# xhuan8/SoccerPlayerShapePose

Hardware: NVIDIA B200
Metric: SMPL meshes/sec fwd+bwd (higher is better)
Workload: dtype f32 (bf16x3 split on tcgen05, fp32 accumulate)

## Files before the change

soccerplayershapepose_b200/csrc/blend_umma.cu:

```cuda
#include <cuda.h>
#include <algorithm>

#include "umma_common.cuh"

namespace b200smpl {

template <int BN>
__global__ void __launch_bounds__(GEMM_THREADS, 1)
umma_gemm2_kernel(const __grid_constant__ GemmOps ops, int split3, int ntiles, int nc8, int slab_begin, int slab_end,
                  int slabs_per_split, float* __restrict__ D, int ldd, long long split_stride) {
  constexpr int BNH = BN / 2;
  constexpr int A_BYTES = BM * BK * 2, B_BYTES = BNH * BK * 2;
  static_assert(B_BYTES % 1024 == 0, "the 128-byte swizzle needs every stage offset 1024-byte aligned");
  constexpr int MAX_STAGES = 6;
  constexpr uint32_t TMEM_COLS = 256;
  const int stage_bytes = (split3 ? 2 : 1) * (A_BYTES + B_BYTES);
  const int nstages = split3 ? 3 : 6;
  extern __shared__ unsigned char smem_dyn[];
  unsigned char* smem = reinterpret_cast<unsigned char*>((reinterpret_cast<uintptr_t>(smem_dyn) + 1023) & ~(uintptr_t)1023);
  uint64_t* full_bar = reinterpret_cast<uint64_t*>(smem + MAX_STAGES * (A_BYTES + B_BYTES));
  uint64_t* peer_full_bar = full_bar + MAX_STAGES;
  uint64_t* empty_bar = peer_full_bar + MAX_STAGES;
  uint64_t* tmem_full_bar = empty_bar + MAX_STAGES;
  uint32_t* tmem_slot = reinterpret_cast<uint32_t*>(tmem_full_bar + 1);
// ... 104 lines not shown
      for (int c0 = 0; c0 < BN; c0 += 32) {
        uint32_t v[32];
        tmem_ld_32x32(tmem_base + ((uint32_t)(q * 32) << 16) + (uint32_t)c0, v);
        float* o = drow + c0;
#pragma unroll
        for (int i = 0; i < 32; i += 4)
          if (c0 + i < BN)
            *reinterpret_cast<uint4*>(o + i) = make_uint4(v[i], v[i + 1], v[i + 2], v[i + 3]);
      }
    } else {
#pragma unroll 1
      for (int c0 = 0; c0 < BN; c0 += 4) *reinterpret_cast<uint4*>(drow + c0) = make_uint4(0u, 0u, 0u, 0u);
    }
  }
  tc_fence_before();
  cluster_sync_all();
  if (warp == 1) {
    tc_fence_after();
    asm volatile("tcgen05.dealloc.cta_group::2.sync.aligned.b32 %0, %1;" ::"r"(tmem_base), "r"(TMEM_COLS) : "memory");
  }
}

constexpr int WS_STAGES = 5;
constexpr int WS_MAX_SLABS = 9;
constexpr int WS_BN = 128;


template <int DUMMY>
__global__ void __launch_bounds__(GEMM_THREADS, 1)
blend_fwd_bs2_kernel(const __grid_constant__ CUtensorMap map_w, const __grid_constant__ CUtensorMap map_f, int pslabs,
                     int ksteps_cs, int ksteps_p, int use_lo, int row0, int mtiles, int ntiles_n,
                     const __grid_constant__ BsWork work, float4* __restrict__ vpB, int nc4) {
  constexpr int SLAB = BM * BK * 2;
  constexpr int KS = BK / UMMA_K;
  constexpr uint32_t TMEM_COLS = 512;
  const int nslab_f = 1 + 2 * pslabs;
  const int nslab_w = 1 + (use_lo ? 2 : 1) * pslabs;
  extern __shared__ unsigned char smem_dyn[];
  unsigned char* smem = reinterpret_cast<unsigned char*>((reinterpret_cast<uintptr_t>(smem_dyn) + 1023) & ~(uintptr_t)1023);
  unsigned char* f_s = smem;
  unsigned char* w_s = smem + WS_MAX_SLABS * SLAB;
  uint64_t* bars = reinterpret_cast<uint64_t*>(w_s + WS_STAGES * SLAB);
  uint64_t* f_full = bars;
  uint64_t* peer_f_full = bars + 1;
  uint64_t* full_bar = bars + 2;
  uint64_t* peer_full_bar = full_bar + WS_STAGES;
  uint64_t* empty_bar = peer_full_bar + WS_STAGES;
  uint64_t* tfull_bar = empty_bar + WS_STAGES;
  uint64_t* tempty_bar = tfull_bar + 2;
  uint32_t* tmem_slot = reinterpret_cast<uint32_t*>(tempty_bar + 2);

  const int warp = threadIdx.x >> 5, lane = threadIdx.x & 31;
  const uint32_t rank = cluster_ctarank();
  const int piece = (int)(blockIdx.x >> 1);
  const int btile = (int)work.bp[piece] * 2 + (int)rank;
  const int wtp_begin = work.w0[piece], wtp_end = work.w1[piece];

  if (warp == 0 && lane == 0) {
    prefetch_tmap(&map_w);
    prefetch_tmap(&map_f);
  }
  if (warp == 1 && lane == 0) {
    mbar_init(f_full, 1);
    mbar_init(peer_f_full, 1);
    for (int i = 0; i < WS_STAGES; ++i) {
      mbar_init(&full_bar[i], 1);
      mbar_init(&peer_full_bar[i], 1);
      mbar_init(&empty_bar[i], 1);
    }
    for (int i = 0; i < 2; ++i) {
      mbar_init(&tfull_bar[i], 1);
      mbar_init(&tempty_bar[i], 8);
    }
    fence_barrier_init();
  }
  if (warp == 1) {
    __syncwarp();
    asm volatile("tcgen05.alloc.cta_group::2.sync.aligned.shared::cta.b32 [%0], %1;" ::"r"(smem_u32(tmem_slot)), "r"(TMEM_COLS)
                 : "memory");
    asm volatile("tcgen05.relinquish_alloc_permit.cta_group::2.sync.aligned;" ::: "memory");
  }
  tc_fence_before();
  cluster_sync_all();
  tc_fence_after();
  const uint32_t tmem_base = *tmem_slot;
  pdl_wait();
  if (threadIdx.x == 0) pdl_trigger();

  if (warp == 0) {
    if (elect_one()) {
      mbar_arrive_expect_tx(f_full, (uint32_t)nslab_f * SLAB);
      for (int s = 0; s < nslab_f; ++s) tma_load_2d(f_s + s * SLAB, &map_f, f_full, s * BK, btile * WS_BN);
    }
    __syncwarp();
    const uint64_t pol_keep = l2_policy_evict_last();
    int stage = 0;
    uint32_t phase = 0;
    for (int wtp = wtp_begin; wtp < wtp_end; ++wtp)
      for (int s = 0; s < nslab_w; ++s) {
        mbar_wait(&empty_bar[stage], phase ^ 1);
        if (elect_one()) {
          mbar_arrive_expect_tx(&full_bar[stage], SLAB);
          tma_load_2d_hint(w_s + stage * SLAB, &map_w, &full_bar[stage], s * BK, row0 + (wtp * 2 + (int)rank) * BM, pol_keep);
        }
        __syncwarp();
        if (++stage == WS_STAGES) { stage = 0; phase ^= 1; }
      }
  } else if (warp == 1) {
    int stage = 0;
    uint32_t phase = 0;
    if (rank == 0) {
      constexpr uint32_t idesc = make_idesc(2 * BM, 2 * WS_BN);
      mbar_wait(f_full, 0);
      mbar_wait(peer_f_full, 0);
      uint32_t tph0 = 0, tph1 = 0;
      int acc = 0;
      for (int wtp = wtp_begin; wtp < wtp_end; ++wtp, acc ^= 1) {
        const uint32_t tph = acc ? tph1 : tph0;
        mbar_wait(&tempty_bar[acc], tph ^ 1);
        if (acc) tph1 ^= 1; else tph0 ^= 1;
        tc_fence_after();
        const uint32_t d_tmem = tmem_base + (uint32_t)(acc * 2 * WS_BN);
        for (int s = 0; s < nslab_w; ++s) {
          mbar_wait(&full_bar[stage], phase);
          mbar_wait(&peer_full_bar[stage], phase);
          tc_fence_after();
          const uint64_t db = make_sw128_desc(smem_u32(w_s + stage * SLAB));
          int ks = ksteps_cs, f0 = 0, f1 = -1;
          if (s > 0) {
            const int j = (s - 1) % pslabs;
            ks = min(KS, ksteps_p - j * KS);
            f0 = 1 + j;
            if (s <= pslabs) f1 = 1 + pslabs + j;
          }
          const uint64_t da0 = make_sw128_desc(smem_u32(f_s + f0 * SLAB));
          const uint64_t da1 = make_sw128_desc(smem_u32(f_s + max(f1, 0) * SLAB));
          if (elect_one()) {
#pragma unroll
            for (int k = 0; k < KS; ++k)
              if (k < ks) umma_bf16_2cta(d_tmem, da0 + 2 * k, db + 2 * k, idesc, (s | k) != 0);
            if (f1 >= 0) {
#pragma unroll
              for (int k = 0; k < KS; ++k)
                if (k < ks) umma_bf16_2cta(d_tmem, da1 + 2 * k, db + 2 * k, idesc, 1u);
            }
            umma_commit_2cta(&empty_bar[stage]);
            if (s == nslab_w - 1) umma_commit_2cta(&tfull_bar[acc]);
          }
          __syncwarp();
          if (++stage == WS_STAGES) { stage = 0; phase ^= 1; }
        }
      }
    } else {
      mbar_wait(f_full, 0);
      if (elect_one()) remote_arrive(peer_f_full, 0);
      __syncwarp();
      for (int wtp = wtp_begin; wtp < wtp_end; ++wtp)
        for (int s = 0; s < nslab_w; ++s) {
          mbar_wait(&full_bar[stage], phase);
          if (elect_one()) remote_arrive(&peer_full_bar[stage], 0);
          __syncwarp();
          if (++stage == WS_STAGES) { stage = 0; phase ^= 1; }
        }
    }
  } else {
    const int q = warp & 3;
    uint32_t tph0 = 0, tph1 = 0;
    int acc = 0;
    for (int wtp = wtp_begin; wtp < wtp_end; ++wtp, acc ^= 1) {
      const uint32_t tph = acc ? tph1 : tph0;
      mbar_wait(&tfull_bar[acc], tph);
      if (acc) tph1 ^= 1; else tph0 ^= 1;
      tc_fence_after();
      if (btile < ntiles_n) {
        const bool live_hi = wtp * 2 + 1 < mtiles;
        float4* colbase = vpB + ((size_t)(btile * 4 + q) * nc4 + ((row0 + wtp * 2 * BM) >> 2)) * 32 + lane;
#pragma unroll 1
        for (int c0 = 0; c0 < 2 * WS_BN; c0 += 32) {
          if (c0 >= WS_BN && !live_hi) continue;
          uint32_t v[32];
          tmem_ld_32x32(tmem_base + ((uint32_t)(q * 32) << 16) + (uint32_t)(acc * 2 * WS_BN + c0), v);
// ... 16 lines not shown
  cluster_sync_all();
  if (warp == 1) {
    tc_fence_after();
    asm volatile("tcgen05.dealloc.cta_group::2.sync.aligned.b32 %0, %1;" ::"r"(tmem_base), "r"(TMEM_COLS) : "memory");
  }
}

typedef CUresult (*EncodeTiledFn)(CUtensorMap*, CUtensorMapDataType, cuuint32_t, void*, const cuuint64_t*,
                                  const cuuint64_t*, const cuuint32_t*, const cuuint32_t*, CUtensorMapInterleave,
                                  CUtensorMapSwizzle, CUtensorMapL2promotion, CUtensorMapFloatOOBfill);

static EncodeTiledFn get_encode_fn() {
  static EncodeTiledFn fn = nullptr;
  if (fn == nullptr) {
    void* p = nullptr;
    cudaDriverEntryPointQueryResult qres;
    if (cudaGetDriverEntryPoint("cuTensorMapEncodeTiled", &p, cudaEnableDefault, &qres) == cudaSuccess &&
        qres == cudaDriverEntryPointSuccess)
      fn = reinterpret_cast<EncodeTiledFn>(p);
  }
  return fn;
}

int make_map(CUtensorMap* map, const void* base, int k_extent, int rows, int pitch_elems, int box_rows) {
  EncodeTiledFn fn = get_encode_fn();
  if (fn == nullptr) return fail(B200SMPL_ERR_CUDA, "cuTensorMapEncodeTiled entry point not available");
  cuuint64_t dims[2] = {(cuuint64_t)k_extent, (cuuint64_t)rows};
  cuuint64_t strides[1] = {(cuuint64_t)pitch_elems * 2};
  cuuint32_t box[2] = {(cuuint32_t)BK, (cuuint32_t)box_rows};
  cuuint32_t estr[2] = {1, 1};
  CUresult r = fn(map, CU_TENSOR_MAP_DATA_TYPE_BFLOAT16, 2, const_cast<void*>(base), dims, strides, box, estr,
                  CU_TENSOR_MAP_INTERLEAVE_NONE, CU_TENSOR_MAP_SWIZZLE_128B, CU_TENSOR_MAP_L2_PROMOTION_L2_256B,
                  CU_TENSOR_MAP_FLOAT_OOB_FILL_NONE);
  if (r != CUDA_SUCCESS) return fail(B200SMPL_ERR_CUDA, "cuTensorMapEncodeTiled failed with code " + std::to_string((int)r));
  return 0;
}

int build_bs_work(int bp_total, int wtp_total, int tpcs, BsWork& work) {
  if (bp_total < 1 || wtp_total < 1) return -1;
  const long long total = (long long)bp_total * wtp_total;
  const int nranges = (int)std::min<long long>(total, std::max(tpcs, bp_total));
  struct Piece { int bp, w0, w1; };
  std::vector<Piece> pieces;
  for (int r = 0; r < nranges; ++r) {
    long long lo = total * r / nranges, hi = total * (r + 1) / nranges;
    while (lo < hi) {
      const int bp = (int)(lo / wtp_total);
      const long long end = std::min<long long>(hi, (long long)(bp + 1) * wtp_total);
      pieces.push_back({bp, (int)(lo - (long long)bp * wtp_total), (int)(end - (long long)bp * wtp_total)});
      lo = end;
    }
  }
  const int rect_chunks = std::max(1, std::min(wtp_total, tpcs / std::max(1, bp_total)));
  const int rect_len = (wtp_total + rect_chunks - 1) / rect_chunks;
  const int flat_len = (int)((total + nranges - 1) / nranges);
  if ((int)pieces.size() > BS_MAX_WORK || rect_len <= flat_len + 1) {
    pieces.clear();
    const int chunks = std::max(1, std::min(rect_chunks, BS_MAX_WORK / bp_total));
    const int wpc = (wtp_total + chunks - 1) / chunks;
    for (int bp = 0; bp < bp_total; ++bp)
      for (int w = 0; w < wtp_total; w += wpc) pieces.push_back({bp, w, std::min(wtp_total, w + wpc)});
    if ((int)pieces.size() > BS_MAX_WORK) return -1;
  }
  std::stable_sort(pieces.begin(), pieces.end(), [](const Piece& a, const Piece& b) { return a.w1 - a.w0 > b.w1 - b.w0; });
  memset(&work, 0, sizeof(work));
  int npieces = 0;
  for (const Piece& pc : pieces) {
    work.bp[npieces] = (uint16_t)pc.bp; work.w0[npieces] = (uint16_t)pc.w0; work.w1[npieces] = (uint16_t)pc.w1;
    ++npieces;
  }
  return npieces;
}

int launch_blend_fwd_umma(const DevModel& m, int mode, const __nv_bfloat16* feat, int S, int Sw, float* vpT,
                          int row_begin, int row_end, int num_sms, cudaStream_t st) {
  const int pslabs = m.fl.pseg / BK;
  const int use_lo = (mode == B200SMPL_MODE_BF16) ? 0 : 1;
  if (1 + 2 * pslabs > WS_MAX_SLABS) return fail(B200SMPL_ERR_INVALID, "feature pitch too large for the resident operand");
  CUtensorMap map_w, map_f;
  int rc;
  if ((rc = make_map(&map_w, m.Wf, m.fl.pitch, m.n_pad, m.fl.pitch, BM))) return rc;
  if ((rc = make_map(&map_f, feat, m.fl.pitch, Sw, m.fl.pitch, WS_BN))) return rc;
  constexpr int smem = (WS_MAX_SLABS + WS_STAGES) * BM * BK * 2 + 1024 + 256;
  auto kern = blend_fwd_bs2_kernel<0>;
  B200_SMEM_ATTR_ONCE(kern, smem);
  const int mtiles = (row_end - row_begin) / BM;
  const int wtp_total = (mtiles + 1) / 2;
  const int ntiles_n = Sw / WS_BN;
  const int bp_total = (ntiles_n + 1) / 2;
  BsWork work;
  const int npieces = build_bs_work(bp_total, wtp_total, std::max(1, num_sms / 2), work);
  if (npieces < 0) return fail(B200SMPL_ERR_INVALID, "slab too wide for the forward GEMM work list");
  cudaLaunchConfig_t cfg;
  memset(&cfg, 0, sizeof(cfg));
  cfg.gridDim = dim3(2 * npieces, 1, 1);
  cfg.blockDim = dim3(GEMM_THREADS, 1, 1);
  cfg.dynamicSmemBytes = smem;
  cfg.stream = st;
  cudaLaunchAttribute attr[2];
  attr[0].id = cudaLaunchAttributeClusterDimension;
  attr[0].val.clusterDim.x = 2;
  attr[0].val.clusterDim.y = 1;
  attr[0].val.clusterDim.z = 1;
  attr[1].id = cudaLaunchAttributeProgrammaticStreamSerialization;
  attr[1].val.programmaticStreamSerializationAllowed = 1;
  cfg.attrs = attr;
  cfg.numAttrs = pdl_enabled() ? 2 : 1;
  LaunchTimer _timer("blend_fwd_umma", st);
  B200_CUDA_TRY(cudaLaunchKernelEx(&cfg, kern, map_w, map_f, pslabs, (m.fl.k_cs + UMMA_K - 1) / UMMA_K,
                                   (NPOSE + UMMA_K - 1) / UMMA_K, use_lo, row_begin, mtiles, ntiles_n, work,
                                   reinterpret_cast<float4*>(vpT), m.n_pad / 4));
  B200_LAUNCH_CHECK("blend_fwd_umma");
  return 0;
}

}
extern "C" int b200smpl_debug_fwd_gemm_worklist(int body_tiles, int row_tiles, int num_sms, uint16_t* out, int capacity) {
  using namespace b200smpl;
  BsWork work;
  const int n = build_bs_work((body_tiles + 1) / 2, (row_tiles + 1) / 2, std::max(1, num_sms / 2), work);
  if (n < 0 || out == nullptr || n > capacity) return n < 0 ? -1 : n;
  for (int c = 0; c < n; ++c) { out[c * 3] = work.bp[c]; out[c * 3 + 1] = work.w0[c]; out[c * 3 + 2] = work.w1[c]; }
  return n;
}
namespace b200smpl {

int blend_bwd_umma_splits(const DevModel& m, int S, int num_sms) {
  const int mtiles = round_up((S + BM - 1) / BM, 2);
  const int slabs = (m.n_rows + BK - 1) / BK;
  int want = std::max(1, num_sms / mtiles);
  want = std::max(1, std::min(want, slabs / 8));
  return want;
}

// ... 52 lines not shown
```

soccerplayershapepose_b200/csrc/fused_fwd.cu:

```cuda
#include <algorithm>

#include "lbs_tiles.cuh"
#include "umma_common.cuh"

namespace b200smpl {

constexpr int FF_BN = 96;
constexpr int FF_BNH = FF_BN / 2;
constexpr int FF_NW = 2;
constexpr int FF_STAGES = 7;
constexpr int FF_STAGE_BYTES = FF_BNH * BK * 2;
constexpr int FF_PS = (NPOSE + BK - 1) / BK;
constexpr int FF_KSP = (NPOSE + UMMA_K - 1) / UMMA_K;
constexpr int FF_MAX_SLABS = 1 + 2 * FF_PS;
constexpr int FF_SLAB = BM * BK * 2;
constexpr int FF_EPI_WARPS = 4 * FF_NW;
constexpr int FF_EPI_WARP0 = 2;
constexpr int FF_THREADS = (FF_EPI_WARP0 + FF_EPI_WARPS) * 32;
constexpr int FF_HV = 8;
constexpr int FF_TR_COL = 2 * FF_BN;
constexpr int FF_WV = TILE_V / 2;
constexpr int FF_PLAN_WORDS = (FF_WV / 8) * 40;
constexpr int FF_TILE_WORDS = ItemShape<FF_HV>::TILE_WORDS;
constexpr int FF_NBARS = 1 + 2 * FF_STAGES + 4 + 2 * FF_EPI_WARPS;
constexpr size_t FF_SMEM = (size_t)FF_MAX_SLABS * FF_SLAB + (size_t)FF_STAGES * FF_STAGE_BYTES +
                           (size_t)FF_EPI_WARPS * (FF_TILE_WORDS + 2 * FF_PLAN_WORDS) * 4 + FF_NBARS * 8 + 16 +
                           1024 ;
static_assert(FF_SMEM <= 232448, "fused forward: shared memory budget");
static_assert(FF_TR_COL + NJ * AELEMS <= 512, "fused forward: tensor memory budget");
static_assert(NJ % FF_NW == 0, "joints split evenly over the warps of a quadrant");

__device__ __forceinline__ void tma_load_2d_pair(void* smem_dst, const CUtensorMap* map, uint64_t* bar, int c0, int c1,
                                                 uint64_t policy) {
  asm volatile(
      "cp.async.bulk.tensor.2d.cta_group::2.shared::cluster.global.mbarrier::complete_tx::bytes.L2::cache_hint [%0], [%1, {%3, %4}], [%2], %5;"
      ::"r"(smem_u32(smem_dst)), "l"(map), "r"(smem_u32(bar) & 0xFEFFFFFFu), "r"(c0), "r"(c1), "l"(policy)
      : "memory");
}

__device__ __forceinline__ void tmem_st_x4(uint32_t taddr, const float4& v) {
  asm volatile("tcgen05.st.sync.aligned.32x32b.x4.b32 [%0], {%1, %2, %3, %4};"
               ::"r"(taddr), "r"(__float_as_uint(v.x)), "r"(__float_as_uint(v.y)), "r"(__float_as_uint(v.z)),
                 "r"(__float_as_uint(v.w))
               : "memory");
}
__device__ __forceinline__ void tmem_wait_st() { asm volatile("tcgen05.wait::st.sync.aligned;" ::: "memory"); }
__device__ __forceinline__ void tmem_ld_12(uint32_t taddr, uint32_t (&r)[12]) {
  asm volatile(
// ... 52 lines not shown
      if (mt & (1u << 21)) load_slot_tm<true>(s.s1, s.zA, tr_base, (mt >> 5) & 31);
      if (mt & (1u << 22)) load_slot_tm<false>(s.s2, s.zB, tr_base, (mt >> 10) & 31);
      if (mt & (1u << 23)) load_slot_tm<true>(s.s3, s.zB, tr_base, (mt >> 15) & 31);
    }
    const f2 px = bc2(P[i * 3]), py = bc2(P[i * 3 + 1]), pz = bc2(P[i * 3 + 2]);
    f2 oxy = txy;
#define B200_SKIN_XY(sl, wk) oxy = fma2(bc2(wk), fma2(sl.c0, px, fma2(sl.c1, py, fma2(sl.c2, pz, sl.t))), oxy);
    B200_SKIN_XY(s.s0, w.x)
    B200_SKIN_XY(s.s1, w.y)
    B200_SKIN_XY(s.s2, w.z)
    B200_SKIN_XY(s.s3, w.w)
#undef B200_SKIN_XY
    f2 oz = fma2(mk2(w.x, w.y), fma2(s.zA.r20, px, fma2(s.zA.r21, py, fma2(s.zA.r22, pz, s.zA.t2))), tz0);
    oz = fma2(mk2(w.z, w.w), fma2(s.zB.r20, px, fma2(s.zB.r21, py, fma2(s.zB.r22, pz, s.zB.t2))), oz);
    o[i * 3] = lo2(oxy); o[i * 3 + 1] = hi2(oxy); o[i * 3 + 2] = lo2(oz) + hi2(oz);
  }
#pragma unroll
  for (int i = 0; i < 3; ++i)
    *reinterpret_cast<float4*>(row_out + i * 4) = make_float4(o[i * 4], o[i * 4 + 1], o[i * 4 + 2], o[i * 4 + 3]);
}

template <bool USE_LO>
__global__ void __launch_bounds__(FF_THREADS, 1)
blend_lbs_fwd_kernel(const __grid_constant__ CUtensorMap map_w, const __grid_constant__ CUtensorMap map_f,
                     int ksteps_cs, int n_pad, int ntiles_n,
                     const __grid_constant__ BsWork work, float4* __restrict__ vpB, int nc4,
                     const float4* __restrict__ A_blk, int b0, int nb, const float* __restrict__ transl,
                     float* __restrict__ verts, int V, int n_vtiles, int vec_ok, const uint32_t* __restrict__ vplan) {
  constexpr int KS = BK / UMMA_K;
  constexpr uint32_t TMEM_COLS = 512;
  using SH = ItemShape<FF_HV>;
  constexpr int PS = FF_PS;
  constexpr int nslab_f = 1 + 2 * PS;
  constexpr int nslab_w = 1 + (USE_LO ? 2 : 1) * PS;
  extern __shared__ __align__(1024) unsigned char smem_dyn[];
  unsigned char* smem = smem_dyn + ((1024u - (smem_u32(smem_dyn) & 1023u)) & 1023u);
  unsigned char* f_s = smem;
  unsigned char* w_s = f_s + FF_MAX_SLABS * FF_SLAB;
  float* tiles = reinterpret_cast<float*>(w_s + FF_STAGES * FF_STAGE_BYTES);
  uint32_t* stashes = reinterpret_cast<uint32_t*>(tiles + FF_EPI_WARPS * FF_TILE_WORDS);
  uint64_t* bars = reinterpret_cast<uint64_t*>(stashes + FF_EPI_WARPS * 2 * FF_PLAN_WORDS);
  uint64_t* f_full = bars;
  uint64_t* full_bar = bars + 1;
  uint64_t* empty_bar = full_bar + FF_STAGES;
  uint64_t* tfull_bar = empty_bar + FF_STAGES;
  uint64_t* tempty_bar = tfull_bar + 2;
  uint64_t* wbars = tempty_bar + 2;
  uint32_t* tmem_slot = reinterpret_cast<uint32_t*>(wbars + 2 * FF_EPI_WARPS);

  const int warp = threadIdx.x >> 5, lane = threadIdx.x & 31;
  const uint32_t rank = cluster_ctarank();
  const int piece = (int)(blockIdx.x >> 1);
  const int btile = (int)work.bp[piece] * 2 + (int)rank;
  const int wt_begin = work.w0[piece], wt_end = work.w1[piece];

  if (warp == 0 && lane == 0) {
    prefetch_tmap(&map_w);
    prefetch_tmap(&map_f);
  }
  if (warp == 1 && lane == 0) {
    mbar_init(f_full, 1);
    for (int i = 0; i < FF_STAGES; ++i) {
      mbar_init(&full_bar[i], 1);
      mbar_init(&empty_bar[i], 1);
    }
    for (int i = 0; i < 2; ++i) {
      mbar_init(&tfull_bar[i], 1);
      mbar_init(&tempty_bar[i], 16);
    }
    for (int i = 0; i < 2 * FF_EPI_WARPS; ++i) mbar_init(&wbars[i], 1);
    fence_barrier_init();
  }
  if (warp == 1) {
    __syncwarp();
    asm volatile("tcgen05.alloc.cta_group::2.sync.aligned.shared::cta.b32 [%0], %1;" ::"r"(smem_u32(tmem_slot)), "r"(TMEM_COLS)
                 : "memory");
    asm volatile("tcgen05.relinquish_alloc_permit.cta_group::2.sync.aligned;" ::: "memory");
  }
  tc_fence_before();
  cluster_sync_all();
  tc_fence_after();
  const uint32_t tmem_base = *tmem_slot;
  pdl_wait();
  if (threadIdx.x == 0) pdl_trigger();

  if (warp < FF_EPI_WARP0) {
  if (warp == 0) {
    const uint64_t pol_keep = l2_policy_evict_last();
    if (elect_one()) {
      if (rank == 0) mbar_arrive_expect_tx(f_full, 2u * (uint32_t)nslab_f * FF_SLAB);
      for (int s = 0; s < nslab_f; ++s) tma_load_2d_pair(f_s + s * FF_SLAB, &map_f, f_full, s * BK, btile * BM, l2_policy_evict_first());
    }
    __syncwarp();
    int stage = 0;
    uint32_t phase = 0;
    for (int wt = wt_begin; wt < wt_end; ++wt)
      for (int s = 0; s < nslab_w; ++s) {
        mbar_wait(&empty_bar[stage], phase ^ 1);
        if (elect_one()) {
          if (rank == 0) mbar_arrive_expect_tx(&full_bar[stage], 2 * FF_STAGE_BYTES);
          tma_load_2d_pair(w_s + stage * FF_STAGE_BYTES, &map_w, &full_bar[stage], s * BK, wt * FF_BN + (int)rank * FF_BNH, pol_keep);
        }
        __syncwarp();
        if (++stage == FF_STAGES) { stage = 0; phase ^= 1; }
      }
  } else if (warp == 1) {
    int stage = 0;
    uint32_t phase = 0;
    if (rank == 0) {
      constexpr uint32_t idesc = make_idesc(2 * BM, FF_BN);
      mbar_wait(f_full, 0);
      const uint64_t da_base = make_sw128_desc(smem_u32(f_s));
      const uint64_t db_base = make_sw128_desc(smem_u32(w_s));
      uint32_t tph0 = 0, tph1 = 0;
      int acc = 0;
      auto slab = [&](uint32_t d_tmem, int ks, int f0, int f1, bool first, uint64_t* tfull) {
        mbar_wait(&full_bar[stage], phase);
        tc_fence_after();
        const uint64_t db = db_base + (uint64_t)(stage * (FF_STAGE_BYTES >> 4));
        if (elect_one()) {
          const uint64_t da0 = da_base + (uint64_t)(f0 * (FF_SLAB >> 4));
#pragma unroll
          for (int k = 0; k < KS; ++k)
            if (k < ks) umma_bf16_2cta(d_tmem, da0 + 2 * k, db + 2 * k, idesc, (first && k == 0) ? 0u : 1u);
          if (f1 >= 0) {
            const uint64_t da1 = da_base + (uint64_t)(f1 * (FF_SLAB >> 4));
#pragma unroll
            for (int k = 0; k < KS; ++k)
              if (k < ks) umma_bf16_2cta(d_tmem, da1 + 2 * k, db + 2 * k, idesc, 1u);
          }
          umma_commit_2cta(&empty_bar[stage]);
          if (tfull != nullptr) umma_commit_2cta(tfull);
        }
        __syncwarp();
        if (++stage == FF_STAGES) { stage = 0; phase ^= 1; }
      };
#pragma unroll 1
      for (int wt = wt_begin; wt < wt_end; ++wt, acc ^= 1) {
        const uint32_t tph = acc ? tph1 : tph0;
        mbar_wait(&tempty_bar[acc], tph ^ 1);
        if (acc) tph1 ^= 1; else tph0 ^= 1;
        tc_fence_after();
        const uint32_t d_tmem = tmem_base + (uint32_t)(acc * FF_BN);
        slab(d_tmem, ksteps_cs, 0, -1, true, nullptr);
#pragma unroll
        for (int j = 0; j < PS; ++j)
          slab(d_tmem, min(KS, FF_KSP - j * KS), 1 + j, 1 + PS + j, false, (!USE_LO && j == PS - 1) ? &tfull_bar[acc] : nullptr);
        if (USE_LO) {
#pragma unroll
          for (int j = 0; j < PS; ++j)
            slab(d_tmem, min(KS, FF_KSP - j * KS), 1 + j, -1, false, j == PS - 1 ? &tfull_bar[acc] : nullptr);
        }
      }
    }
  }
  } else {
    const int e = warp - FF_EPI_WARP0, q = warp & 3, r3 = e >> 2;
    float* tile = tiles + e * FF_TILE_WORDS;
    float* my_row = tile + lane * SH::HROW;
    uint32_t* stash = stashes + e * 2 * FF_PLAN_WORDS;
    uint64_t* wbar = wbars + e * 2;
    const bool live = btile < ntiles_n;
    const int g = btile * 4 + q;
    const uint32_t lane_base = tmem_base + ((uint32_t)(q * 32) << 16);
    const uint32_t tr_base = lane_base + FF_TR_COL;
    const bool skin = verts != nullptr;
    if (live && skin) {
      const float4* ap = A_blk + (size_t)g * (NJ * 3 * 32) + lane;
#pragma unroll 1
      for (int j = r3 * (NJ / FF_NW); j < (r3 + 1) * (NJ / FF_NW); ++j) {
        const float4 x0 = ap[(j * 3) * 32], x1 = ap[(j * 3 + 1) * 32], x2 = ap[(j * 3 + 2) * 32];
        tmem_st_x4(tr_base + j * AELEMS, x0);
        tmem_st_x4(tr_base + j * AELEMS + 4, x1);
        tmem_st_x4(tr_base + j * AELEMS + 8, x2);
      }
// ... 82 lines not shown
          float4* o = colbase + (size_t)(c0 >> 2) * 32;
#pragma unroll
          for (int i = 0; i < 6; ++i)
            if (row_w + c0 + 4 * i < n_pad)
              o[i * 32] = make_float4(__uint_as_float(v[4 * i]), __uint_as_float(v[4 * i + 1]),
                                      __uint_as_float(v[4 * i + 2]), __uint_as_float(v[4 * i + 3]));
        }
      }
    }
  }
  tc_fence_before();
  cluster_sync_all();
  if (warp == 1) {
    tc_fence_after();
    asm volatile("tcgen05.dealloc.cta_group::2.sync.aligned.b32 %0, %1;" ::"r"(tmem_base), "r"(TMEM_COLS) : "memory");
  }
}

int launch_blend_lbs_fwd(const DevModel& m, int mode, const __nv_bfloat16* feat, int S, int Sw, float* vpT,
                         const float* A_blk, int b0, int nb, const float* transl, float* verts, int num_sms,
                         cudaStream_t st) {
  (void)S;
  const bool use_lo = mode != B200SMPL_MODE_BF16;
  if (m.fl.pseg != FF_PS * BK) return fail(B200SMPL_ERR_INVALID, "fused forward: unexpected pose segment width");
  if (m.n_virt0 != m.ntiles * FF_BN) return fail(B200SMPL_ERR_INVALID, "fused forward: vertex tiles must be 96 rows");
  CUtensorMap map_w, map_f;
  int rc;
  if ((rc = make_map(&map_w, m.Wf, m.fl.pitch, m.n_pad, m.fl.pitch, FF_BNH))) return rc;
  if ((rc = make_map(&map_f, feat, m.fl.pitch, Sw, m.fl.pitch, BM))) return rc;
  auto kern = use_lo ? blend_lbs_fwd_kernel<true> : blend_lbs_fwd_kernel<false>;
  B200_SMEM_ATTR_ONCE(blend_lbs_fwd_kernel<true>, FF_SMEM);
  B200_SMEM_ATTR_ONCE(blend_lbs_fwd_kernel<false>, FF_SMEM);
  const int wt_total = (m.n_pad + FF_BN - 1) / FF_BN;
  const int ntiles_n = Sw / BM;
  const int bp_total = (ntiles_n + 1) / 2;
  BsWork work;
  const int npieces = build_bs_work(bp_total, wt_total, std::max(1, num_sms / 2), work);
  if (npieces < 0) return fail(B200SMPL_ERR_INVALID, "slab too wide for the fused forward work list");
  const int vec_ok = (verts != nullptr && (m.V & 1) == 0 && (reinterpret_cast<uintptr_t>(verts) & 7) == 0) ? 1 : 0;
  cudaLaunchConfig_t cfg;
  memset(&cfg, 0, sizeof(cfg));
  cfg.gridDim = dim3(2 * npieces, 1, 1);
  cfg.blockDim = dim3(FF_THREADS, 1, 1);
  cfg.dynamicSmemBytes = FF_SMEM;
  cfg.stream = st;
  cudaLaunchAttribute attr[2];
  attr[0].id = cudaLaunchAttributeClusterDimension;
  attr[0].val.clusterDim.x = 2;
  attr[0].val.clusterDim.y = 1;
  attr[0].val.clusterDim.z = 1;
  attr[1].id = cudaLaunchAttributeProgrammaticStreamSerialization;
  attr[1].val.programmaticStreamSerializationAllowed = 1;
  cfg.attrs = attr;
  cfg.numAttrs = pdl_enabled() ? 2 : 1;
  LaunchTimer _timer("blend_lbs_fwd", st);
  B200_CUDA_TRY(cudaLaunchKernelEx(&cfg, kern, map_w, map_f, (m.fl.k_cs + UMMA_K - 1) / UMMA_K, m.n_pad, ntiles_n, work,
                                   reinterpret_cast<float4*>(vpT), m.n_pad / 4, reinterpret_cast<const float4*>(A_blk), b0, nb,
                                   transl, verts, m.V, m.ntiles, vec_ok, m.vplan));
  B200_LAUNCH_CHECK("blend_lbs_fwd");
  return 0;
}

}
```

soccerplayershapepose_b200/csrc/umma_common.cuh:

```cuda
#pragma once

#include <cuda.h>

#include "skin_common.cuh"

namespace b200smpl {

constexpr int BM = 128;
constexpr int BK = 64;
constexpr int UMMA_K = 16;
constexpr int GEMM_THREADS = 192;

struct GemmOps {
  const __nv_bfloat16* dvp_hi;
  const __nv_bfloat16* dvp_lo;
  CUtensorMap wb_hi, wb_lo;
};

__device__ __forceinline__ uint32_t smem_u32(const void* p) { return (uint32_t)__cvta_generic_to_shared(p); }

__device__ __forceinline__ void mbar_arrive_expect_tx(uint64_t* bar, uint32_t bytes) {
  asm volatile("mbarrier.arrive.expect_tx.shared::cta.b64 _, [%0], %1;" ::"r"(smem_u32(bar)), "r"(bytes) : "memory");
}
__device__ __forceinline__ void fence_barrier_init() { asm volatile("fence.mbarrier_init.release.cluster;" ::: "memory"); }
// ... 79 lines not shown
  return (1u << 4) | (1u << 7) | (1u << 10) | ((uint32_t)(N >> 3) << 17) | ((uint32_t)(M >> 4) << 24);
}

__device__ __forceinline__ void umma_bf16_2cta(uint32_t tmem_d, uint64_t desc_a, uint64_t desc_b, uint32_t idesc,
                                               uint32_t accumulate) {
  asm volatile(
      "{\n\t.reg .pred p;\n\t"
      "setp.ne.b32 p, %4, 0;\n\t"
      "tcgen05.mma.cta_group::2.kind::f16 [%0], %1, %2, %3, p;\n\t}"
      ::"r"(tmem_d), "l"(desc_a), "l"(desc_b), "r"(idesc), "r"(accumulate)
      : "memory");
}
__device__ __forceinline__ void umma_commit_2cta(uint64_t* bar) {
  asm volatile("tcgen05.commit.cta_group::2.mbarrier::arrive::one.shared::cluster.multicast::cluster.b64 [%0], %1;"
               ::"r"(smem_u32(bar)), "h"((uint16_t)3)
               : "memory");
}
__device__ __forceinline__ void remote_arrive(uint64_t* local_bar, uint32_t cta) {
  uint32_t remote;
  asm volatile("mapa.shared::cluster.u32 %0, %1, %2;" : "=r"(remote) : "r"(smem_u32(local_bar)), "r"(cta));
  asm volatile("mbarrier.arrive.relaxed.cluster.shared::cluster.b64 _, [%0];" ::"r"(remote) : "memory");
}

constexpr int BS_MAX_WORK = 160;
struct BsWork {
  uint16_t bp[BS_MAX_WORK], w0[BS_MAX_WORK], w1[BS_MAX_WORK];
};
int build_bs_work(int bp_total, int wtp_total, int tpcs, BsWork& work);
int make_map(CUtensorMap* map, const void* base, int k_extent, int rows, int pitch_elems, int box_rows);

}
```

Before: 6.942 million.

## Load pose-segment K tails as narrow unswizzled tiles instead of padded slabs

The forward blend GEMMs used to load and multiply each pose segment padded up to a whole 64-wide K slab. Now each segment is split into full swizzled tiles plus one 16-wide tail tile, loaded through separate no-swizzle tensor maps. The tail is packed into the same pipeline stage as the preceding tile, and the resident feature operand shrinks accordingly. This cuts TMA bytes, shared memory and MMA issue for the padding columns, and frees smem for more weight stages in the fused kernel. The cost is more TMA descriptors and instructions per stage and more complex descriptor and offset arithmetic.

```diff
diff --git a/soccerplayershapepose_b200/csrc/blend_umma.cu b/soccerplayershapepose_b200/csrc/blend_umma.cu
--- a/soccerplayershapepose_b200/csrc/blend_umma.cu
+++ b/soccerplayershapepose_b200/csrc/blend_umma.cu
@@ -150,25 +150,28 @@
 }
 
 constexpr int WS_STAGES = 5;
-constexpr int WS_MAX_SLABS = 9;
 constexpr int WS_BN = 128;
+constexpr int WS_SLOT = BM * (BK + FWD_TAIL_W) * 2;
+constexpr int WS_RES = BM * FWD_RES_ROW_BYTES;
+constexpr int WS_SMEM = WS_RES + WS_STAGES * WS_SLOT + 1024 + 256;
+static_assert(WS_RES % 1024 == 0 && WS_SLOT % 1024 == 0, "the 128-byte swizzle needs 1024-byte aligned tiles");
+static_assert(WS_SMEM <= 232448, "forward GEMM: shared memory budget");
 
 
 template <int DUMMY>
 __global__ void __launch_bounds__(GEMM_THREADS, 1)
-blend_fwd_bs2_kernel(const __grid_constant__ CUtensorMap map_w, const __grid_constant__ CUtensorMap map_f, int pslabs,
-                     int ksteps_cs, int ksteps_p, int use_lo, int row0, int mtiles, int ntiles_n,
+blend_fwd_bs2_kernel(const __grid_constant__ CUtensorMap map_w, const __grid_constant__ CUtensorMap map_wt,
+                     const __grid_constant__ CUtensorMap map_f, const __grid_constant__ CUtensorMap map_ft,
+                     int ksteps_cs, int use_lo, int row0, int mtiles, int ntiles_n,
                      const __grid_constant__ BsWork work, float4* __restrict__ vpB, int nc4) {
-  constexpr int SLAB = BM * BK * 2;
   constexpr int KS = BK / UMMA_K;
   constexpr uint32_t TMEM_COLS = 512;
-  const int nslab_f = 1 + 2 * pslabs;
-  const int nslab_w = 1 + (use_lo ? 2 : 1) * pslabs;
+  const int nkt_w = use_lo ? FWD_KT : FWD_KT_BF16;
   extern __shared__ unsigned char smem_dyn[];
   unsigned char* smem = reinterpret_cast<unsigned char*>((reinterpret_cast<uintptr_t>(smem_dyn) + 1023) & ~(uintptr_t)1023);
   unsigned char* f_s = smem;
-  unsigned char* w_s = smem + WS_MAX_SLABS * SLAB;
-  uint64_t* bars = reinterpret_cast<uint64_t*>(w_s + WS_STAGES * SLAB);
+  unsigned char* w_s = smem + WS_RES;
+  uint64_t* bars = reinterpret_cast<uint64_t*>(w_s + WS_STAGES * WS_SLOT);
   uint64_t* f_full = bars;
   uint64_t* peer_f_full = bars + 1;
   uint64_t* full_bar = bars + 2;
@@ -186,7 +189,9 @@
 
   if (warp == 0 && lane == 0) {
     prefetch_tmap(&map_w);
+    prefetch_tmap(&map_wt);
     prefetch_tmap(&map_f);
+    prefetch_tmap(&map_ft);
   }
   if (warp == 1 && lane == 0) {
     mbar_init(f_full, 1);
@@ -217,23 +222,41 @@
 
   if (warp == 0) {
     if (elect_one()) {
-      mbar_arrive_expect_tx(f_full, (uint32_t)nslab_f * SLAB);
-      for (int s = 0; s < nslab_f; ++s) tma_load_2d(f_s + s * SLAB, &map_f, f_full, s * BK, btile * WS_BN);
+      mbar_arrive_expect_tx(f_full, (uint32_t)WS_RES);
+      for (int t = 0; t < FWD_KT; ++t) {
+        unsigned char* dst = f_s + fwd_kt_res_off(t, BM);
+        if (fwd_kt_tail(t)) {
+          tma_load_2d(dst, &map_ft, f_full, fwd_kt_col(t), btile * WS_BN);
+          tma_load_2d(dst + BM * 16, &map_ft, f_full, fwd_kt_col(t) + FWD_TAIL_BOX, btile * WS_BN);
+        } else {
+          tma_load_2d(dst, &map_f, f_full, fwd_kt_col(t), btile * WS_BN);
+        }
+      }
     }
     __syncwarp();
     const uint64_t pol_keep = l2_policy_evict_last();
     int stage = 0;
     uint32_t phase = 0;
-    for (int wtp = wtp_begin; wtp < wtp_end; ++wtp)
-      for (int s = 0; s < nslab_w; ++s) {
+    for (int wtp = wtp_begin; wtp < wtp_end; ++wtp) {
+      const int mrow = row0 + (wtp * 2 + (int)rank) * BM;
+      for (int t = 0; t < nkt_w; ++t) {
+        const bool tail = fwd_kt_tail(t + 1);
         mbar_wait(&empty_bar[stage], phase ^ 1);
         if (elect_one()) {
-          mbar_arrive_expect_tx(&full_bar[stage], SLAB);
-          tma_load_2d_hint(w_s + stage * SLAB, &map_w, &full_bar[stage], s * BK, row0 + (wtp * 2 + (int)rank) * BM, pol_keep);
+          unsigned char* slot = w_s + stage * WS_SLOT;
+          mbar_arrive_expect_tx(&full_bar[stage], BM * (BK + (tail ? FWD_TAIL_W : 0)) * 2);
+          tma_load_2d_hint(slot, &map_w, &full_bar[stage], fwd_kt_col(t), mrow, pol_keep);
+          if (tail) {
+            unsigned char* dt = slot + BM * BK * 2;
+            tma_load_2d_hint(dt, &map_wt, &full_bar[stage], fwd_kt_col(t + 1), mrow, pol_keep);
+            tma_load_2d_hint(dt + BM * 16, &map_wt, &full_bar[stage], fwd_kt_col(t + 1) + FWD_TAIL_BOX, mrow, pol_keep);
+          }
         }
         __syncwarp();
+        t += tail;
         if (++stage == WS_STAGES) { stage = 0; phase ^= 1; }
       }
+    }
   } else if (warp == 1) {
     int stage = 0;
     uint32_t phase = 0;
@@ -241,6 +264,7 @@
       constexpr uint32_t idesc = make_idesc(2 * BM, 2 * WS_BN);
       mbar_wait(f_full, 0);
       mbar_wait(peer_f_full, 0);
+      const uint32_t f_addr = smem_u32(f_s);
       uint32_t tph0 = 0, tph1 = 0;
       int acc = 0;
       for (int wtp = wtp_begin; wtp < wtp_end; ++wtp, acc ^= 1) {
@@ -249,42 +273,47 @@
         if (acc) tph1 ^= 1; else tph0 ^= 1;
         tc_fence_after();
         const uint32_t d_tmem = tmem_base + (uint32_t)(acc * 2 * WS_BN);
-        for (int s = 0; s < nslab_w; ++s) {
+        for (int t = 0; t < nkt_w; ++t) {
+          const int tail = fwd_kt_tail(t + 1) ? 1 : 0;
           mbar_wait(&full_bar[stage], phase);
           mbar_wait(&peer_full_bar[stage], phase);
           tc_fence_after();
-          const uint64_t db = make_sw128_desc(smem_u32(w_s + stage * SLAB));
-          int ks = ksteps_cs, f0 = 0, f1 = -1;
-          if (s > 0) {
-            const int j = (s - 1) % pslabs;
-            ks = min(KS, ksteps_p - j * KS);
-            f0 = 1 + j;
-            if (s <= pslabs) f1 = 1 + pslabs + j;
+          const uint32_t slot = smem_u32(w_s + stage * WS_SLOT);
+          const bool issue = elect_one();
+#pragma unroll 1
+          for (int u = 0; u <= tail; ++u) {
+            const int tt = t + u, f0 = fwd_kt_f0(tt), f1 = fwd_kt_f1(tt);
+            const int ks = tt == 0 ? ksteps_cs : fwd_kt_width(tt) / UMMA_K;
+            const uint64_t db = fwd_kt_desc(tt, slot + (uint32_t)(u * BM * BK * 2), BM);
+            const uint64_t da0 = fwd_kt_desc(f0, f_addr + (uint32_t)fwd_kt_res_off(f0, BM), BM);
+            const uint64_t da1 = fwd_kt_desc(max(f1, 0), f_addr + (uint32_t)fwd_kt_res_off(max(f1, 0), BM), BM);
+            if (issue) {
+#pragma unroll
+              for (int k = 0; k < KS; ++k)
+                if (k < ks) umma_bf16_2cta(d_tmem, da0 + 2 * k, db + 2 * k, idesc, (tt | k) != 0);
+              if (f1 >= 0) {
+#pragma unroll
+                for (int k = 0; k < KS; ++k)
+                  if (k < ks) umma_bf16_2cta(d_tmem, da1 + 2 * k, db + 2 * k, idesc, 1u);
+              }
+            }
           }
-          const uint64_t da0 = make_sw128_desc(smem_u32(f_s + f0 * SLAB));
-          const uint64_t da1 = make_sw128_desc(smem_u32(f_s + max(f1, 0) * SLAB));
-          if (elect_one()) {
-#pragma unroll
-            for (int k = 0; k < KS; ++k)
-              if (k < ks) umma_bf16_2cta(d_tmem, da0 + 2 * k, db + 2 * k, idesc, (s | k) != 0);
-            if (f1 >= 0) {
-#pragma unroll
-              for (int k = 0; k < KS; ++k)
-                if (k < ks) umma_bf16_2cta(d_tmem, da1 + 2 * k, db + 2 * k, idesc, 1u);
-            }
+          if (issue) {
             umma_commit_2cta(&empty_bar[stage]);
-            if (s == nslab_w - 1) umma_commit_2cta(&tfull_bar[acc]);
+            if (t + tail == nkt_w - 1) umma_commit_2cta(&tfull_bar[acc]);
           }
           __syncwarp();
+          t += tail;
           if (++stage == WS_STAGES) { stage = 0; phase ^= 1; }
         }
       }
     } else {
+      const int nstage_w = use_lo ? FWD_WIDE_TILES : 1 + FWD_SEG_WIDE;
       mbar_wait(f_full, 0);
       if (elect_one()) remote_arrive(peer_f_full, 0);
       __syncwarp();
       for (int wtp = wtp_begin; wtp < wtp_end; ++wtp)
-        for (int s = 0; s < nslab_w; ++s) {
+        for (int s = 0; s < nstage_w; ++s) {
           mbar_wait(&full_bar[stage], phase);
           if (elect_one()) remote_arrive(&peer_full_bar[stage], 0);
           __syncwarp();
@@ -347,18 +376,24 @@
   return fn;
 }
 
-int make_map(CUtensorMap* map, const void* base, int k_extent, int rows, int pitch_elems, int box_rows) {
+int make_map(CUtensorMap* map, const void* base, int k_extent, int rows, int pitch_elems, int box_rows, int box_k) {
+  if (box_k != BK && box_k != FWD_TAIL_BOX) return fail(B200SMPL_ERR_INVALID, "make_map: unsupported box width");
   EncodeTiledFn fn = get_encode_fn();
   if (fn == nullptr) return fail(B200SMPL_ERR_CUDA, "cuTensorMapEncodeTiled entry point not available");
   cuuint64_t dims[2] = {(cuuint64_t)k_extent, (cuuint64_t)rows};
   cuuint64_t strides[1] = {(cuuint64_t)pitch_elems * 2};
-  cuuint32_t box[2] = {(cuuint32_t)BK, (cuuint32_t)box_rows};
+  cuuint32_t box[2] = {(cuuint32_t)box_k, (cuuint32_t)box_rows};
   cuuint32_t estr[2] = {1, 1};
   CUresult r = fn(map, CU_TENSOR_MAP_DATA_TYPE_BFLOAT16, 2, const_cast<void*>(base), dims, strides, box, estr,
-                  CU_TENSOR_MAP_INTERLEAVE_NONE, CU_TENSOR_MAP_SWIZZLE_128B, CU_TENSOR_MAP_L2_PROMOTION_L2_256B,
-                  CU_TENSOR_MAP_FLOAT_OOB_FILL_NONE);
+                  CU_TENSOR_MAP_INTERLEAVE_NONE, box_k == BK ? CU_TENSOR_MAP_SWIZZLE_128B : CU_TENSOR_MAP_SWIZZLE_NONE,
+                  CU_TENSOR_MAP_L2_PROMOTION_L2_256B, CU_TENSOR_MAP_FLOAT_OOB_FILL_NONE);
   if (r != CUDA_SUCCESS) return fail(B200SMPL_ERR_CUDA, "cuTensorMapEncodeTiled failed with code " + std::to_string((int)r));
   return 0;
+}
+
+int make_fwd_maps(CUtensorMap* wide, CUtensorMap* tail, const void* base, int rows, int pitch_elems, int box_rows) {
+  int rc = make_map(wide, base, pitch_elems, rows, pitch_elems, box_rows, BK);
+  return rc ? rc : make_map(tail, base, pitch_elems, rows, pitch_elems, box_rows, FWD_TAIL_BOX);
 }
 
 int build_bs_work(int bp_total, int wtp_total, int tpcs, BsWork& work) {
@@ -399,16 +434,15 @@
 
 int launch_blend_fwd_umma(const DevModel& m, int mode, const __nv_bfloat16* feat, int S, int Sw, float* vpT,
                           int row_begin, int row_end, int num_sms, cudaStream_t st) {
-  const int pslabs = m.fl.pseg / BK;
   const int use_lo = (mode == B200SMPL_MODE_BF16) ? 0 : 1;
-  if (1 + 2 * pslabs > WS_MAX_SLABS) return fail(B200SMPL_ERR_INVALID, "feature pitch too large for the resident operand");
-  CUtensorMap map_w, map_f;
+  if (m.fl.pseg != FWD_PSEG || m.fl.off_p1 != FWD_PSEG + BK)
+    return fail(B200SMPL_ERR_INVALID, "forward GEMM: unexpected feature layout");
+  CUtensorMap map_w, map_wt, map_f, map_ft;
   int rc;
-  if ((rc = make_map(&map_w, m.Wf, m.fl.pitch, m.n_pad, m.fl.pitch, BM))) return rc;
-  if ((rc = make_map(&map_f, feat, m.fl.pitch, Sw, m.fl.pitch, WS_BN))) return rc;
-  constexpr int smem = (WS_MAX_SLABS + WS_STAGES) * BM * BK * 2 + 1024 + 256;
+  if ((rc = make_fwd_maps(&map_w, &map_wt, m.Wf, m.n_pad, m.fl.pitch, BM))) return rc;
+  if ((rc = make_fwd_maps(&map_f, &map_ft, feat, Sw, m.fl.pitch, WS_BN))) return rc;
   auto kern = blend_fwd_bs2_kernel<0>;
-  B200_SMEM_ATTR_ONCE(kern, smem);
+  B200_SMEM_ATTR_ONCE(kern, WS_SMEM);
   const int mtiles = (row_end - row_begin) / BM;
   const int wtp_total = (mtiles + 1) / 2;
   const int ntiles_n = Sw / WS_BN;
@@ -420,7 +454,7 @@
   memset(&cfg, 0, sizeof(cfg));
   cfg.gridDim = dim3(2 * npieces, 1, 1);
   cfg.blockDim = dim3(GEMM_THREADS, 1, 1);
-  cfg.dynamicSmemBytes = smem;
+  cfg.dynamicSmemBytes = WS_SMEM;
   cfg.stream = st;
   cudaLaunchAttribute attr[2];
   attr[0].id = cudaLaunchAttributeClusterDimension;
@@ -432,9 +466,8 @@
   cfg.attrs = attr;
   cfg.numAttrs = pdl_enabled() ? 2 : 1;
   LaunchTimer _timer("blend_fwd_umma", st);
-  B200_CUDA_TRY(cudaLaunchKernelEx(&cfg, kern, map_w, map_f, pslabs, (m.fl.k_cs + UMMA_K - 1) / UMMA_K,
-                                   (NPOSE + UMMA_K - 1) / UMMA_K, use_lo, row_begin, mtiles, ntiles_n, work,
-                                   reinterpret_cast<float4*>(vpT), m.n_pad / 4));
+  B200_CUDA_TRY(cudaLaunchKernelEx(&cfg, kern, map_w, map_wt, map_f, map_ft, (m.fl.k_cs + UMMA_K - 1) / UMMA_K, use_lo,
+                                   row_begin, mtiles, ntiles_n, work, reinterpret_cast<float4*>(vpT), m.n_pad / 4));
   B200_LAUNCH_CHECK("blend_fwd_umma");
   return 0;
 }
diff --git a/soccerplayershapepose_b200/csrc/fused_fwd.cu b/soccerplayershapepose_b200/csrc/fused_fwd.cu
--- a/soccerplayershapepose_b200/csrc/fused_fwd.cu
+++ b/soccerplayershapepose_b200/csrc/fused_fwd.cu
@@ -8,12 +8,10 @@
 constexpr int FF_BN = 96;
 constexpr int FF_BNH = FF_BN / 2;
 constexpr int FF_NW = 2;
-constexpr int FF_STAGES = 7;
-constexpr int FF_STAGE_BYTES = FF_BNH * BK * 2;
-constexpr int FF_PS = (NPOSE + BK - 1) / BK;
-constexpr int FF_KSP = (NPOSE + UMMA_K - 1) / UMMA_K;
-constexpr int FF_MAX_SLABS = 1 + 2 * FF_PS;
-constexpr int FF_SLAB = BM * BK * 2;
+constexpr int FF_STAGES = 8;
+constexpr int FF_STAGE_BYTES = 8192;
+static_assert(FF_BNH * (BK + FWD_TAIL_W) * 2 <= FF_STAGE_BYTES, "fused forward: a stage holds a tile and a tail");
+constexpr int FF_RES = BM * FWD_RES_ROW_BYTES;
 constexpr int FF_EPI_WARPS = 4 * FF_NW;
 constexpr int FF_EPI_WARP0 = 2;
 constexpr int FF_THREADS = (FF_EPI_WARP0 + FF_EPI_WARPS) * 32;
@@ -23,7 +21,7 @@
 constexpr int FF_PLAN_WORDS = (FF_WV / 8) * 40;
 constexpr int FF_TILE_WORDS = ItemShape<FF_HV>::TILE_WORDS;
 constexpr int FF_NBARS = 1 + 2 * FF_STAGES + 4 + 2 * FF_EPI_WARPS;
-constexpr size_t FF_SMEM = (size_t)FF_MAX_SLABS * FF_SLAB + (size_t)FF_STAGES * FF_STAGE_BYTES +
+constexpr size_t FF_SMEM = (size_t)FF_RES + (size_t)FF_STAGES * FF_STAGE_BYTES +
                            (size_t)FF_EPI_WARPS * (FF_TILE_WORDS + 2 * FF_PLAN_WORDS) * 4 + FF_NBARS * 8 + 16 +
                            1024 ;
 static_assert(FF_SMEM <= 232448, "fused forward: shared memory budget");
@@ -122,21 +120,19 @@
 
 template <bool USE_LO>
 __global__ void __launch_bounds__(FF_THREADS, 1)
-blend_lbs_fwd_kernel(const __grid_constant__ CUtensorMap map_w, const __grid_constant__ CUtensorMap map_f,
-                     int ksteps_cs, int n_pad, int ntiles_n,
+blend_lbs_fwd_kernel(const __grid_constant__ CUtensorMap map_w, const __grid_constant__ CUtensorMap map_wt,
+                     const __grid_constant__ CUtensorMap map_f, const __grid_constant__ CUtensorMap map_ft, int ksteps_cs, int n_pad, int ntiles_n,
                      const __grid_constant__ BsWork work, float4* __restrict__ vpB, int nc4,
                      const float4* __restrict__ A_blk, int b0, int nb, const float* __restrict__ transl,
                      float* __restrict__ verts, int V, int n_vtiles, int vec_ok, const uint32_t* __restrict__ vplan) {
   constexpr int KS = BK / UMMA_K;
   constexpr uint32_t TMEM_COLS = 512;
   using SH = ItemShape<FF_HV>;
-  constexpr int PS = FF_PS;
-  constexpr int nslab_f = 1 + 2 * PS;
-  constexpr int nslab_w = 1 + (USE_LO ? 2 : 1) * PS;
+  constexpr int NKT = USE_LO ? FWD_KT : FWD_KT_BF16;
   extern __shared__ __align__(1024) unsigned char smem_dyn[];
   unsigned char* smem = smem_dyn + ((1024u - (smem_u32(smem_dyn) & 1023u)) & 1023u);
   unsigned char* f_s = smem;
-  unsigned char* w_s = f_s + FF_MAX_SLABS * FF_SLAB;
+  unsigned char* w_s = f_s + FF_RES;
   float* tiles = reinterpret_cast<float*>(w_s + FF_STAGES * FF_STAGE_BYTES);
   uint32_t* stashes = reinterpret_cast<uint32_t*>(tiles + FF_EPI_WARPS * FF_TILE_WORDS);
   uint64_t* bars = reinterpret_cast<uint64_t*>(stashes + FF_EPI_WARPS * 2 * FF_PLAN_WORDS);
@@ -156,7 +152,9 @@
 
   if (warp == 0 && lane == 0) {
     prefetch_tmap(&map_w);
+    prefetch_tmap(&map_wt);
     prefetch_tmap(&map_f);
+    prefetch_tmap(&map_ft);
   }
   if (warp == 1 && lane == 0) {
     mbar_init(f_full, 1);
@@ -188,20 +186,38 @@
   if (warp == 0) {
     const uint64_t pol_keep = l2_policy_evict_last();
     if (elect_one()) {
-      if (rank == 0) mbar_arrive_expect_tx(f_full, 2u * (uint32_t)nslab_f * FF_SLAB);
-      for (int s = 0; s < nslab_f; ++s) tma_load_2d_pair(f_s + s * FF_SLAB, &map_f, f_full, s * BK, btile * BM, l2_policy_evict_first());
+      const uint64_t pol_stream = l2_policy_evict_first();
+      if (rank == 0) mbar_arrive_expect_tx(f_full, 2u * (uint32_t)FF_RES);
+      for (int t = 0; t < FWD_KT; ++t) {
+        unsigned char* dst = f_s + fwd_kt_res_off(t, BM);
+        if (fwd_kt_tail(t)) {
+          tma_load_2d_pair(dst, &map_ft, f_full, fwd_kt_col(t), btile * BM, pol_stream);
+          tma_load_2d_pair(dst + BM * 16, &map_ft, f_full, fwd_kt_col(t) + FWD_TAIL_BOX, btile * BM, pol_stream);
+        } else {
+          tma_load_2d_pair(dst, &map_f, f_full, fwd_kt_col(t), btile * BM, pol_stream);
+        }
+      }
     }
     __syncwarp();
     int stage = 0;
     uint32_t phase = 0;
     for (int wt = wt_begin; wt < wt_end; ++wt)
-      for (int s = 0; s < nslab_w; ++s) {
+      for (int t = 0; t < NKT; ++t) {
+        const bool tail = fwd_kt_tail(t + 1);
         mbar_wait(&empty_bar[stage], phase ^ 1);
         if (elect_one()) {
-          if (rank == 0) mbar_arrive_expect_tx(&full_bar[stage], 2 * FF_STAGE_BYTES);
-          tma_load_2d_pair(w_s + stage * FF_STAGE_BYTES, &map_w, &full_bar[stage], s * BK, wt * FF_BN + (int)rank * FF_BNH, pol_keep);
+          unsigned char* dst = w_s + stage * FF_STAGE_BYTES;
+          const int mrow = wt * FF_BN + (int)rank * FF_BNH;
+          if (rank == 0) mbar_arrive_expect_tx(&full_bar[stage], 2 * FF_BNH * (BK + (tail ? FWD_TAIL_W : 0)) * 2);
+          tma_load_2d_pair(dst, &map_w, &full_bar[stage], fwd_kt_col(t), mrow, pol_keep);
+          if (tail) {
+            unsigned char* dt = dst + FF_BNH * BK * 2;
+            tma_load_2d_pair(dt, &map_wt, &full_bar[stage], fwd_kt_col(t + 1), mrow, pol_keep);
+            tma_load_2d_pair(dt + FF_BNH * 16, &map_wt, &full_bar[stage], fwd_kt_col(t + 1) + FWD_TAIL_BOX, mrow, pol_keep);
+          }
         }
         __syncwarp();
+        t += tail;
         if (++stage == FF_STAGES) { stage = 0; phase ^= 1; }
       }
   } else if (warp == 1) {
@@ -210,25 +226,32 @@
     if (rank == 0) {
       constexpr uint32_t idesc = make_idesc(2 * BM, FF_BN);
       mbar_wait(f_full, 0);
-      const uint64_t da_base = make_sw128_desc(smem_u32(f_s));
+      const uint32_t f_addr = smem_u32(f_s);
       const uint64_t db_base = make_sw128_desc(smem_u32(w_s));
+      const uint64_t dbt_base = make_nosw_desc(smem_u32(w_s), FF_BNH * 16, 128);
       uint32_t tph0 = 0, tph1 = 0;
       int acc = 0;
-      auto slab = [&](uint32_t d_tmem, int ks, int f0, int f1, bool first, uint64_t* tfull) {
+      auto tile_mma = [&](uint32_t d_tmem, int t, uint64_t db) {
+        const int ks = t == 0 ? ksteps_cs : fwd_kt_width(t) / UMMA_K;
+        const int f0 = fwd_kt_f0(t), f1 = fwd_kt_f1(t);
+        const uint64_t da0 = fwd_kt_desc(f0, f_addr + (uint32_t)fwd_kt_res_off(f0, BM), BM);
+#pragma unroll
+        for (int k = 0; k < KS; ++k)
+          if (k < ks) umma_bf16_2cta(d_tmem, da0 + 2 * k, db + 2 * k, idesc, (t == 0 && k == 0) ? 0u : 1u);
+        if (f1 >= 0) {
+          const uint64_t da1 = fwd_kt_desc(f1, f_addr + (uint32_t)fwd_kt_res_off(f1, BM), BM);
+#pragma unroll
+          for (int k = 0; k < KS; ++k)
+            if (k < ks) umma_bf16_2cta(d_tmem, da1 + 2 * k, db + 2 * k, idesc, 1u);
+        }
+      };
+      auto stage_mma = [&](uint32_t d_tmem, int t, uint64_t* tfull) {
         mbar_wait(&full_bar[stage], phase);
         tc_fence_after();
-        const uint64_t db = db_base + (uint64_t)(stage * (FF_STAGE_BYTES >> 4));
+        const uint64_t off = (uint64_t)(stage * (FF_STAGE_BYTES >> 4));
         if (elect_one()) {
-          const uint64_t da0 = da_base + (uint64_t)(f0 * (FF_SLAB >> 4));
-#pragma unroll
-          for (int k = 0; k < KS; ++k)
-            if (k < ks) umma_bf16_2cta(d_tmem, da0 + 2 * k, db + 2 * k, idesc, (first && k == 0) ? 0u : 1u);
-          if (f1 >= 0) {
-            const uint64_t da1 = da_base + (uint64_t)(f1 * (FF_SLAB >> 4));
-#pragma unroll
-            for (int k = 0; k < KS; ++k)
-              if (k < ks) umma_bf16_2cta(d_tmem, da1 + 2 * k, db + 2 * k, idesc, 1u);
-          }
+          tile_mma(d_tmem, t, db_base + off);
+          if (fwd_kt_tail(t + 1)) tile_mma(d_tmem, t + 1, dbt_base + off + (uint64_t)((FF_BNH * BK * 2) >> 4));
           umma_commit_2cta(&empty_bar[stage]);
           if (tfull != nullptr) umma_commit_2cta(tfull);
         }
@@ -242,15 +265,9 @@
         if (acc) tph1 ^= 1; else tph0 ^= 1;
         tc_fence_after();
         const uint32_t d_tmem = tmem_base + (uint32_t)(acc * FF_BN);
-        slab(d_tmem, ksteps_cs, 0, -1, true, nullptr);
-#pragma unroll
-        for (int j = 0; j < PS; ++j)
-          slab(d_tmem, min(KS, FF_KSP - j * KS), 1 + j, 1 + PS + j, false, (!USE_LO && j == PS - 1) ? &tfull_bar[acc] : nullptr);
-        if (USE_LO) {
-#pragma unroll
-          for (int j = 0; j < PS; ++j)
-            slab(d_tmem, min(KS, FF_KSP - j * KS), 1 + j, -1, false, j == PS - 1 ? &tfull_bar[acc] : nullptr);
-        }
+#pragma unroll
+        for (int t = 0; t < NKT; ++t)
+          if (!fwd_kt_tail(t)) stage_mma(d_tmem, t, t + (fwd_kt_tail(t + 1) ? 1 : 0) == NKT - 1 ? &tfull_bar[acc] : nullptr);
       }
     }
   }
@@ -379,12 +396,13 @@
                          cudaStream_t st) {
   (void)S;
   const bool use_lo = mode != B200SMPL_MODE_BF16;
-  if (m.fl.pseg != FF_PS * BK) return fail(B200SMPL_ERR_INVALID, "fused forward: unexpected pose segment width");
+  if (m.fl.pseg != FWD_PSEG || m.fl.off_p1 != FWD_PSEG + BK)
+    return fail(B200SMPL_ERR_INVALID, "fused forward: unexpected feature layout");
   if (m.n_virt0 != m.ntiles * FF_BN) return fail(B200SMPL_ERR_INVALID, "fused forward: vertex tiles must be 96 rows");
-  CUtensorMap map_w, map_f;
+  CUtensorMap map_w, map_wt, map_f, map_ft;
   int rc;
-  if ((rc = make_map(&map_w, m.Wf, m.fl.pitch, m.n_pad, m.fl.pitch, FF_BNH))) return rc;
-  if ((rc = make_map(&map_f, feat, m.fl.pitch, Sw, m.fl.pitch, BM))) return rc;
+  if ((rc = make_fwd_maps(&map_w, &map_wt, m.Wf, m.n_pad, m.fl.pitch, FF_BNH))) return rc;
+  if ((rc = make_fwd_maps(&map_f, &map_ft, feat, Sw, m.fl.pitch, BM))) return rc;
   auto kern = use_lo ? blend_lbs_fwd_kernel<true> : blend_lbs_fwd_kernel<false>;
   B200_SMEM_ATTR_ONCE(blend_lbs_fwd_kernel<true>, FF_SMEM);
   B200_SMEM_ATTR_ONCE(blend_lbs_fwd_kernel<false>, FF_SMEM);
@@ -411,7 +429,7 @@
   cfg.attrs = attr;
   cfg.numAttrs = pdl_enabled() ? 2 : 1;
   LaunchTimer _timer("blend_lbs_fwd", st);
-  B200_CUDA_TRY(cudaLaunchKernelEx(&cfg, kern, map_w, map_f, (m.fl.k_cs + UMMA_K - 1) / UMMA_K, m.n_pad, ntiles_n, work,
+  B200_CUDA_TRY(cudaLaunchKernelEx(&cfg, kern, map_w, map_wt, map_f, map_ft, (m.fl.k_cs + UMMA_K - 1) / UMMA_K, m.n_pad, ntiles_n, work,
                                    reinterpret_cast<float4*>(vpT), m.n_pad / 4, reinterpret_cast<const float4*>(A_blk), b0, nb,
                                    transl, verts, m.V, m.ntiles, vec_ok, m.vplan));
   B200_LAUNCH_CHECK("blend_lbs_fwd");
diff --git a/soccerplayershapepose_b200/csrc/umma_common.cuh b/soccerplayershapepose_b200/csrc/umma_common.cuh
--- a/soccerplayershapepose_b200/csrc/umma_common.cuh
+++ b/soccerplayershapepose_b200/csrc/umma_common.cuh
@@ -125,11 +125,41 @@
   asm volatile("mbarrier.arrive.relaxed.cluster.shared::cluster.b64 _, [%0];" ::"r"(remote) : "memory");
 }
 
+constexpr int FWD_PSEG = (NPOSE + BK - 1) / BK * BK;
+constexpr int FWD_SEG_WIDE = NPOSE / BK;
+constexpr int FWD_SEG_TILES = FWD_SEG_WIDE + 1;
+constexpr int FWD_TAIL_W = UMMA_K;
+constexpr int FWD_TAIL_BOX = 8;
+constexpr int FWD_KT = 1 + 2 * FWD_SEG_TILES;
+constexpr int FWD_KT_BF16 = 1 + FWD_SEG_TILES;
+constexpr int FWD_WIDE_TILES = 1 + 2 * FWD_SEG_WIDE;
+constexpr int FWD_RES_ROW_BYTES = FWD_WIDE_TILES * BK * 2 + 2 * FWD_TAIL_W * 2;
+static_assert(NPOSE > FWD_SEG_WIDE * BK && NPOSE <= FWD_SEG_WIDE * BK + FWD_TAIL_W, "the tail is one K step");
+
+__host__ __device__ constexpr bool fwd_kt_tail(int t) { return t > 0 && (t - 1) % FWD_SEG_TILES == FWD_SEG_WIDE; }
+__host__ __device__ constexpr int fwd_kt_width(int t) { return fwd_kt_tail(t) ? FWD_TAIL_W : BK; }
+__host__ __device__ constexpr int fwd_kt_col(int t) {
+  return t == 0 ? 0 : BK + (t - 1) / FWD_SEG_TILES * FWD_PSEG + (t - 1) % FWD_SEG_TILES * BK;
+}
+__host__ __device__ constexpr int fwd_kt_f0(int t) { return t <= FWD_SEG_TILES ? t : t - FWD_SEG_TILES; }
+__host__ __device__ constexpr int fwd_kt_f1(int t) { return t >= 1 && t <= FWD_SEG_TILES ? t + FWD_SEG_TILES : -1; }
+__host__ __device__ constexpr int fwd_kt_res_off(int t, int rows) {
+  return rows * (fwd_kt_tail(t) ? FWD_WIDE_TILES * BK * 2 + (t - 1) / FWD_SEG_TILES * FWD_TAIL_W * 2
+                                : (t - (t > 0 ? (t - 1) / FWD_SEG_TILES : 0)) * BK * 2);
+}
+__device__ __forceinline__ uint64_t fwd_kt_desc(int t, uint32_t addr, int rows) {
+  return fwd_kt_tail(t) ? make_nosw_desc(addr, (uint32_t)rows * 16u, 128u) : make_sw128_desc(addr);
+}
+static_assert(fwd_kt_col(FWD_SEG_TILES) == BK + FWD_SEG_WIDE * BK && fwd_kt_col(FWD_KT - 1) == BK + FWD_PSEG + FWD_SEG_WIDE * BK,
+              "tails sit at the end of the used columns of each segment");
+static_assert(fwd_kt_res_off(FWD_KT - 1, 1) + FWD_TAIL_W * 2 == FWD_RES_ROW_BYTES, "resident layout");
+
 constexpr int BS_MAX_WORK = 160;
 struct BsWork {
   uint16_t bp[BS_MAX_WORK], w0[BS_MAX_WORK], w1[BS_MAX_WORK];
 };
 int build_bs_work(int bp_total, int wtp_total, int tpcs, BsWork& work);
-int make_map(CUtensorMap* map, const void* base, int k_extent, int rows, int pitch_elems, int box_rows);
+int make_map(CUtensorMap* map, const void* base, int k_extent, int rows, int pitch_elems, int box_rows, int box_k = BK);
+int make_fwd_maps(CUtensorMap* wide, CUtensorMap* tail, const void* base, int rows, int pitch_elems, int box_rows);
 
 }
```

After: 7.003 million (median of 6 runs). About the same (+0.9%).
